# ai4co/rl4co

Measured on NVIDIA H100. Metric: node-selections/sec TSP-100 AM rollout, higher is better.
Workload: dtype f32

## Files before the change

### rl4co_b200/csrc/rollout_impl.cuh

```cuda
#pragma once
#include "co_common.cuh"

namespace co {

#define CO_MODE_GREEDY 0
#define CO_MODE_SAMPLE 1
#define CO_MODE_EVALUATE 2

template <int SPL>
struct Cfg {
  static constexpr int NS = 32 * SPL;
  static constexpr int NW = SPL;
  static constexpr int MINB = SPL == 4 ? 1 : (SPL == 2 ? 2 : 3);
};

constexpr int TILE_LD = 20;

template <int SPL>
struct Smem {
  float ptab[(32 * SPL + 1) * E];
  float qfix[E];
  float wcap[E];
  float hfirst[E];
  float tile[8][32 * TILE_LD];
  alignas(16) float oh[8][D];
  alignas(16) float part[8][32 * SPL];
  alignas(16) float zbuf[2][32 * SPL];
  alignas(16) uint2 red[4];
  alignas(16) float lps[32];
  float dem[32 * SPL];
  float lim[32 * SPL];
  float2 loc[32 * SPL];
  unsigned char order[32 * SPL];
  unsigned char rank_of[32 * SPL];
  alignas(16) float wdyn[3 * E];
  alignas(16) float pwk[32 * SPL * 8 + 8];
};

__device__ __forceinline__ float ex2(float x) {
  float y;
  asm("ex2.approx.ftz.f32 %0, %1;" : "=f"(y) : "f"(x));
  return y;
}
__device__ __forceinline__ float lg2(float x) {
  float y;
  asm("lg2.approx.ftz.f32 %0, %1;" : "=f"(y) : "f"(x));
  return y;
}
__device__ __forceinline__ unsigned fkey(float f) {
  unsigned u = __float_as_uint(f);
  return u ^ ((u >> 31) ? 0xffffffffu : 0x80000000u);
}
__device__ __forceinline__ float funkey(unsigned k) {
  return __uint_as_float(k ^ ((k >> 31) ? 0x80000000u : 0xffffffffu));
}

__device__ __forceinline__ float warp_sum_fixed(float x) {
  constexpr float S = 16777216.f;
  const unsigned hi = __float2uint_rz(x * S);
  const float rem = fmaf(x, S, -(float)hi);
  const unsigned lo = __float2uint_rz(rem * S);
  const unsigned Hs = __reduce_add_sync(FULL, hi), Ls = __reduce_add_sync(FULL, lo);
  return fmaf((float)Ls, 1.0f / (S * S), (float)Hs * (1.0f / S));
}

static __device__ __noinline__ void first_node_gemv(const float* __restrict__ w_first, const float* hfirst, float* qfix, int tid) {
  const int e = tid >> 1, half = tid & 1;
  const float4* wr = reinterpret_cast<const float4*>(w_first + (size_t)e * E + 64 * half);
  const float4* hv = reinterpret_cast<const float4*>(hfirst + 64 * half);
  float s0 = 0.f, s1 = 0.f;
#pragma unroll
  for (int c = 0; c < 16; c += 2) {
    const float4 w0 = __ldg(wr + c), x0 = hv[c], w1 = __ldg(wr + c + 1), x1 = hv[c + 1];
    s0 = fmaf(w0.x, x0.x, s0); s0 = fmaf(w0.y, x0.y, s0); s0 = fmaf(w0.z, x0.z, s0); s0 = fmaf(w0.w, x0.w, s0);
    s1 = fmaf(w1.x, x1.x, s1); s1 = fmaf(w1.y, x1.y, s1); s1 = fmaf(w1.z, x1.z, s1); s1 = fmaf(w1.w, x1.w, s1);
  }
  float sacc = s0 + s1;
  sacc += __shfl_xor_sync(FULL, sacc, 1);
  if (half == 0) qfix[e] += sacc;
}

__device__ __forceinline__ float dist2_fma(float2 a, float2 b) {
  const float dx = a.x - b.x, dy = a.y - b.y;
  return sqrtf(fmaf(dy, dy, dx * dx));
}

template <int ENV>
__device__ __forceinline__ bool feasible(int n, bool visbit, float d, float used, float thr, int cur, bool anyfeas) {
  if (ENV == CO_ENV_TSP) return !visbit;
  if (ENV == CO_ENV_OP) return (n == 0) || (!visbit && !anyfeas && !(d > thr));
  if (ENV == CO_ENV_PCTSP) return (n == 0) ? !((used < 1.0f) && anyfeas) : (!visbit && d == 0.0f);
  if (n == 0) return !(cur == 0 && anyfeas);
  if (ENV == CO_ENV_SDVRP) return !visbit && !(d == 0.0f) && !(used >= thr);
  return !visbit && !((d + used) > thr);
}

template <int SPL, int ENV, int MODE, int CWB>
__global__ void __launch_bounds__(256, Cfg<SPL>::MINB) rollout_kernel(const co_rollout_args A) {
  using C = Cfg<SPL>;
  constexpr int NS = C::NS, NW = C::NW;
  constexpr int CW = CWB * E;
  constexpr int CUR_BLK = CWB - 1;
  constexpr bool first_table = (ENV == CO_ENV_TSP) && (CWB == 5);
  constexpr bool VRP = (ENV != CO_ENV_TSP);
  constexpr bool SD = (ENV == CO_ENV_SDVRP);
  constexpr bool OP = (ENV == CO_ENV_OP);
  constexpr bool PC = (ENV == CO_ENV_PCTSP);
  constexpr float LOG2E = 1.4426950408889634f, LN2 = 0.6931471805599453f;
  extern __shared__ __align__(16) unsigned char smem_raw[];
  Smem<SPL>& sm = *reinterpret_cast<Smem<SPL>*>(smem_raw);

  const int tid = threadIdx.x, lane = tid & 31, h = tid >> 5;
  const int N = A.N, B_inst = A.B_inst, S = A.num_starts, T_max = A.T_max;
  const int B_traj = B_inst * S;
  const bool forced_start = (S > 1) && (A.flags & CO_ROLLOUT_FORCED_START);
  const bool philox = (A.noise == nullptr);
  const bool sel_warp = h < NW;
  const bool lp_warp = h == NW;
  const int nL = sel_warp ? tid : NS - 1;
  const int nG = SPL * lane;
  const float clip = A.tanh_clipping, inv_temp = 1.0f / A.temperature;
  const float Zb = clip * inv_temp;
  float* tile = sm.tile[h];

  float2 Kr[SPL][8], Vr[SPL][8], Lr[SPL][8];

  for (int b = blockIdx.x; b < B_inst; b += gridDim.x) {
    __syncthreads();
    const float* crow = A.cache + (size_t)b * N * CW;
#pragma unroll
    for (int k = 0; k < SPL; ++k) {
      const int n = nG + k;
      if (n < N) {
        const float4* ks = reinterpret_cast<const float4*>(crow + (size_t)n * CW + 0 * E + h * D);
        const float4* vs = reinterpret_cast<const float4*>(crow + (size_t)n * CW + 1 * E + h * D);
        const float4* ls = reinterpret_cast<const float4*>(crow + (size_t)n * CW + 2 * E + h * D);
#pragma unroll
        for (int c = 0; c < 4; ++c) {
          const float4 kv = __ldg(ks + c), vv = __ldg(vs + c), lv = __ldg(ls + c);
          Kr[k][2 * c] = make_float2(kv.x, kv.y); Kr[k][2 * c + 1] = make_float2(kv.z, kv.w);
          Vr[k][2 * c] = make_float2(vv.x, vv.y); Vr[k][2 * c + 1] = make_float2(vv.z, vv.w);
          Lr[k][2 * c] = make_float2(lv.x, lv.y); Lr[k][2 * c + 1] = make_float2(lv.z, lv.w);
        }
      } else {
#pragma unroll
        for (int j = 0; j < 8; ++j) {
          Kr[k][j] = make_float2(0.f, 0.f); Vr[k][j] = make_float2(0.f, 0.f); Lr[k][j] = make_float2(0.f, 0.f);
        }
      }
    }
    for (int idx = tid; idx < N * (E / 4); idx += 256) {
      const int n = idx >> 5, c = idx & 31;
      const uint32_t dst = (uint32_t)__cvta_generic_to_shared(reinterpret_cast<float4*>(sm.ptab + n * E) + c);
      asm volatile("cp.async.cg.shared.global [%0], [%1], 16;" ::"r"(dst),
                   "l"(reinterpret_cast<const float4*>(crow + (size_t)n * CW + CUR_BLK * E) + c) : "memory");
    }
    asm volatile("cp.async.commit_group;" ::: "memory");
    if (tid < E) {
      sm.ptab[NS * E + tid] = 0.f;
      sm.wcap[tid] = VRP ? A.w_capacity[tid] : 0.f;
    }
    if (tid < NS) {
      sm.loc[tid] = (tid < N) ? reinterpret_cast<const float2*>(A.locs)[(size_t)b * N + tid] : make_float2(0.f, 0.f);
      sm.dem[tid] = (VRP && tid >= 1 && tid < N) ? A.demand[(size_t)b * (N - 1) + tid - 1] : 0.f;
      if (OP || PC) sm.lim[tid] = (tid < N) ? A.node_limit[(size_t)b * N + tid] : 0.f;
    }
    if (SD) {
      for (int i = tid; i < 3 * E; i += 256) sm.wdyn[i] = A.dyn_w[i];
    }
    const float cap = (VRP && A.vehicle_capacity) ? A.vehicle_capacity[b] : 1.0f;
    const float thr = SD ? cap : cap + 1e-5f;
    asm volatile("cp.async.wait_group 0;" ::: "memory");
    __syncthreads();
    if (SD) {
      for (int i = tid; i < (NS + 1) * 8; i += 256) {
        const int n = i >> 3, hh = i & 7;
        float acc = 0.f;
        if (n < N) {
#pragma unroll
          for (int c = 0; c < D; ++c) acc = fmaf(sm.ptab[n * E + hh * D + c], sm.wdyn[hh * D + c], acc);
        }
        sm.pwk[i] = acc;
      }
      __syncthreads();
    }
    if (ENV == CO_ENV_CVRP) {
      if (tid >= 1 && tid < N) {
        const float d = sm.dem[tid];
        int rank = 0;
        for (int m = 1; m < N; ++m) {
          const float dm = sm.dem[m];
          rank += (dm < d || (dm == d && m < tid)) ? 1 : 0;
        }
        sm.order[rank] = (unsigned char)tid;
        sm.rank_of[tid] = (unsigned char)rank;
      }
      __syncthreads();
    }
    float dmk0[SPL];
    float2 lck[SPL];
#pragma unroll
    for (int k = 0; k < SPL; ++k) {
      dmk0[k] = OP ? sm.lim[nG + k] : sm.dem[nG + k];
      lck[k] = OP ? sm.loc[nG + k] : make_float2(0.f, 0.f);
    }
    const float dL0 = OP ? sm.lim[nL] : sm.dem[nL];
    const float2 lcL = OP ? sm.loc[nL] : make_float2(0.f, 0.f);
    auto head_dot = [&](const float* vec, float (&out)[SPL]) {
      const float4* vp = reinterpret_cast<const float4*>(vec + h * D);
      float2 a2[SPL];
#pragma unroll
      for (int k = 0; k < SPL; ++k) a2[k] = make_float2(0.f, 0.f);
#pragma unroll
      for (int c = 0; c < 4; ++c) {
        const float4 x = vp[c];
#pragma unroll
        for (int k = 0; k < SPL; ++k) {
          a2[k] = ffma2(make_float2(x.x, x.y), Kr[k][2 * c], a2[k]);
          a2[k] = ffma2(make_float2(x.z, x.w), Kr[k][2 * c + 1], a2[k]);
        }
      }
#pragma unroll
      for (int k = 0; k < SPL; ++k) out[k] = a2[k].x + a2[k].y;
    };
    auto add_first = [&](int a_first) {
      if (first_table) {
        if (tid < E) sm.qfix[tid] += __ldg(crow + (size_t)a_first * CW + 3 * E + tid);
      } else {
        if (tid < E) sm.hfirst[tid] = __ldg(A.node_emb + ((size_t)b * N + a_first) * E + tid);
        __syncthreads();
        first_node_gemv(A.w_first, sm.hfirst, sm.qfix, tid);
      }
    };
    float WK[SPL], FK[SPL];
#pragma unroll
    for (int k = 0; k < SPL; ++k) { WK[k] = 0.f; FK[k] = 0.f; }
    if (VRP) head_dot(sm.wcap, WK);
    float WKW = 0.f, wv_d = 0.f;
    if (SD) {
#pragma unroll
      for (int c = 0; c < D; ++c) WKW = fmaf(sm.wcap[h * D + c], sm.wdyn[h * D + c], WKW);
      wv_d = sm.wdyn[E + h * D + (lane & 15)];
    }
    if (!(A.flags & CO_ROLLOUT_NO_PREFETCH) && b + (int)gridDim.x < B_inst) {
      const char* nxt = reinterpret_cast<const char*>(A.cache + (size_t)(b + gridDim.x) * N * CW);
      for (int i = tid; i < N * 16; i += 256) {
        const int n = i >> 4, blk = (i >> 2) & 3, line = i & 3;
        const size_t off = ((size_t)n * CW + (blk < 3 ? blk : CUR_BLK) * E) * 4 + ((size_t)line << 7);
        asm volatile("prefetch.global.L2 [%0];" ::"l"(nxt + off));
      }
    }

    for (int s = 0; s < S; ++s) {
      const int traj = s * B_inst + b;
      int64_t* act_row = A.actions_out + (size_t)traj * T_max;
      float* lp_row = A.logp_out + (size_t)traj * T_max;
      uint32_t mybits = (!sel_warp || nL >= N) ? 0x100u : 0u;
#pragma unroll
      for (int k = 0; k < SPL; ++k) mybits |= (nG + k >= N) ? (1u << k) : 0u;
      int cur = (ENV == CO_ENV_TSP) ? NS : 0;
      int prev = 0, first = 0, t = 0, dstep = 0, nvis = 0;
      uint32_t rmask[SPL];
#pragma unroll
      for (int k = 0; k < SPL; ++k) {
        const int lo = 32 * k, nc = N - 1;
        rmask[k] = (nc >= lo + 32) ? 0u : (nc <= lo ? 0xffffffffu : (0xffffffffu << (nc - lo)));
      }
      float used = 0.f, dist = 0.f;
      bool anyfeas = false, done = false, depot_seen = false;
      float dmk[SPL], dL = dL0;
#pragma unroll
      for (int k = 0; k < SPL; ++k) dmk[k] = dmk0[k];
      int nrem = 0;
      int pend_a = -1;
      float pend_d = 0.f, FKW = 0.f;
      float ll = 0.f;
      float pen = 0.f;
      if (SD && s > 0 && tid < NS) sm.dem[tid] = (tid >= 1 && tid < N) ? A.demand[(size_t)b * (N - 1) + tid - 1] : 0.f;
      __syncthreads();
      if (tid < E) {
        float g = A.graph_ctx ? A.graph_ctx[(size_t)b * E + tid] : 0.f;
        if (ENV == CO_ENV_TSP && !forced_start) g += A.q_placeholder[tid];
        sm.qfix[tid] = g;
      }

      auto env_step = [&](int a) {
        if (!SD) {
          const unsigned dd = (unsigned)(a - nG);
          mybits |= (dd < (unsigned)SPL) ? (1u << dd) : 0u;
          mybits |= (a == nL) ? 0x100u : 0u;
        }
        if (!OP && h == 0) {
          const float2 pa = sm.loc[a], pp = sm.loc[prev];
          const float dx = pa.x - pp.x, dy = pa.y - pp.y;
          if (VRP || t != 0) dist += sqrtf(dx * dx + dy * dy);
        }
        if (ENV == CO_ENV_TSP) {
          if (t == 0) first = a;
        } else if (OP) {
          used = used + dist2_fma(sm.loc[a], sm.loc[prev]);
          if (h == 0) dist += sm.dem[a];
          depot_seen = depot_seen || (a == 0);
        } else if (PC) {
          used = used + sm.dem[a];
          if (h == 0) pen += sm.lim[a];
          nvis += (a != 0) ? 1 : 0;
          depot_seen = depot_seen || (a == 0);
        } else if (SD) {
          const float d_a = sm.dem[a];
          const float delivered = fminf(d_a, cap - used);
          used = (used + delivered) * (a != 0 ? 1.0f : 0.0f);
          const float d_new = d_a + (-delivered);
#pragma unroll
          for (int k = 0; k < SPL; ++k) dmk[k] = (a == nG + k) ? d_new : dmk[k];
          dL = (a == nL) ? d_new : dL;
          nrem += ((d_new > 0.f) ? 1 : 0) - ((d_a > 0.f) ? 1 : 0);
          pend_a = a; pend_d = d_new;
          anyfeas = (nrem > 0) && !(used >= cap);
        } else {
          used = (used + sm.dem[a == 0 ? 1 : a]) * (a != 0 ? 1.0f : 0.0f);
          nvis += (a != 0 || !depot_seen) ? 1 : 0;
          depot_seen = depot_seen || (a == 0);
          if (a != 0) {
            const int r = sm.rank_of[a];
#pragma unroll
            for (int k = 0; k < SPL; ++k) rmask[k] |= ((r >> 5) == k) ? (1u << (r & 31)) : 0u;
          }
          int pmin = NS;
#pragma unroll
          for (int k = SPL - 1; k >= 0; --k) {
            const uint32_t z = ~rmask[k];
            if (z) pmin = 32 * k + __ffs(z) - 1;
          }
          anyfeas = (pmin < N - 1) && !((sm.dem[sm.order[pmin < N - 1 ? pmin : 0]] + used) > thr);
        }
        prev = a; cur = a; ++t;
        done = (ENV == CO_ENV_TSP) ? (t >= N) : ((OP || PC) ? (a == 0 && t > 1) : (SD ? (nrem == 0) : (nvis >= N)));
      };
      auto logp_of = [&](int buf, int a_sel, int t_out) {
        const float* zb = sm.zbuf[buf];
        float sacc = 0.f;
#pragma unroll
        for (int k = 0; k < SPL; ++k) sacc += ex2((zb[nG + k] - Zb) * LOG2E);
        sm.lps[lane] = sacc;
        __syncwarp();
        const float4* lq = reinterpret_cast<const float4*>(sm.lps);
        const float4 q0 = lq[0], q1 = lq[1], q2 = lq[2], q3 = lq[3], q4 = lq[4], q5 = lq[5], q6 = lq[6], q7 = lq[7];
        const float t0 = ((q0.x + q0.y) + (q0.z + q0.w)) + ((q1.x + q1.y) + (q1.z + q1.w));
        const float t1 = ((q2.x + q2.y) + (q2.z + q2.w)) + ((q3.x + q3.y) + (q3.z + q3.w));
        const float t2 = ((q4.x + q4.y) + (q4.z + q4.w)) + ((q5.x + q5.y) + (q5.z + q5.w));
        const float t3 = ((q6.x + q6.y) + (q6.z + q6.w)) + ((q7.x + q7.y) + (q7.z + q7.w));
        sacc = (t0 + t1) + (t2 + t3);
        __syncwarp();
        const float lp = (zb[a_sel] - Zb) - lg2(sacc) * LN2;
        if (lane == 0) {
          lp_row[t_out] = lp;
          ll += lp;
        }
      };

      if (SD) {
        for (int n = 1; n < N; ++n) nrem += (sm.dem[n] > 0.f) ? 1 : 0;
        anyfeas = (nrem > 0) && !(used >= cap);
        done = (nrem == 0);
      }
      if (forced_start) {
        const int a0 = (s % A.num_loc) + (VRP ? 1 : 0);
        if (tid == 0) { act_row[0] = a0; lp_row[0] = 0.f; }
        env_step(a0);
        if (ENV == CO_ENV_TSP) {
          __syncthreads();
          add_first(a0);
        }
      } else if (ENV == CO_ENV_CVRP) {
        anyfeas = !((sm.dem[sm.order[0]] + used) > thr);
      }
      __syncthreads();
      head_dot(sm.qfix, FK);
      if (SD) {
#pragma unroll
        for (int c = 0; c < D; ++c) FKW = fmaf(sm.qfix[h * D + c], sm.wdyn[h * D + c], FKW);
      }

      while (!done && t < T_max) {
        int forced = 0;
        float gum = 0.f;
        if (MODE == CO_MODE_EVALUATE) forced = (int)A.forced_actions[(size_t)traj * T_max + t];
        if (MODE == CO_MODE_SAMPLE && tid < N) {
          const float q = philox ? philox_exp1(A.seed, A.offset, traj, dstep, tid)
                                 : A.noise[((size_t)dstep * B_traj + traj) * N + tid];
          gum = -logf(q);
        }

        {
          const float4* pr = reinterpret_cast<const float4*>(sm.ptab + cur * E + h * D);
          const float rem = PC ? fmaxf(cap - used, 0.0f) : cap - used;
          float2 sc2[SPL];
#pragma unroll
          for (int k = 0; k < SPL; ++k) sc2[k] = make_float2(0.f, 0.f);
#pragma unroll
          for (int c = 0; c < 4; ++c) {
            const float4 p = pr[c];
#pragma unroll
            for (int k = 0; k < SPL; ++k) {
              sc2[k] = ffma2(make_float2(p.x, p.y), Kr[k][2 * c], sc2[k]);
              sc2[k] = ffma2(make_float2(p.z, p.w), Kr[k][2 * c + 1], sc2[k]);
            }
          }
          float sc[SPL], m = -INFINITY;
          bool fz[SPL];
          const float qwk = SD ? fmaf(rem, WKW, sm.pwk[cur * 8 + h] + FKW) : 0.f;
          const float2 pcur = OP ? sm.loc[cur] : make_float2(0.f, 0.f);
#pragma unroll
          for (int k = 0; k < SPL; ++k) {
            fz[k] = OP ? feasible<ENV>(nG + k, (mybits >> k) & 1u, used + dist2_fma(lck[k], pcur), used, dmk[k], cur, depot_seen)
                    : PC ? feasible<ENV>(nG + k, (mybits >> k) & 1u, depot_seen ? 1.0f : 0.0f, used, thr, cur, nvis < N - 1)
                         : feasible<ENV>(nG + k, (mybits >> k) & 1u, dmk[k], used, thr, cur, anyfeas);
            float dot = (sc2[k].x + sc2[k].y) + FK[k];
            if (VRP) dot = fmaf(rem, WK[k], dot);
            if (SD) dot = fmaf(dmk[k], qwk, dot);
            sc[k] = fz[k] ? dot * (0.25f * LOG2E) : -INFINITY;
            m = fmaxf(m, sc[k]);
          }
          m = funkey(__reduce_max_sync(FULL, fkey(m)));
          float2 acc[8];
          float esum = 0.f, sed = 0.f;
#pragma unroll
          for (int j = 0; j < 8; ++j) acc[j] = make_float2(0.f, 0.f);
#pragma unroll
          for (int k = 0; k < SPL; ++k) {
            const float e = fz[k] ? ex2(sc[k] - m) : 0.f;
            esum += e;
            if (SD) sed = fmaf(e, dmk[k], sed);
            const float2 e2 = make_float2(e, e);
#pragma unroll
            for (int j = 0; j < 8; ++j) acc[j] = ffma2(e2, Vr[k][j], acc[j]);
          }
          float4* trow = reinterpret_cast<float4*>(tile + lane * TILE_LD);
#pragma unroll
          for (int c = 0; c < 4; ++c) trow[c] = make_float4(acc[2 * c].x, acc[2 * c].y, acc[2 * c + 1].x, acc[2 * c + 1].y);
          if (SD) sed = warp_sum(sed);
          __syncwarp();
          const int d = lane & 15, half = lane >> 4;
          float s0 = 0.f, s1 = 0.f, s2 = 0.f, s3 = 0.f;
#pragma unroll
          for (int r = 0; r < 16; r += 4) {
            s0 += tile[(16 * half + ((r + 0 + 4 * half) & 15)) * TILE_LD + d];
            s1 += tile[(16 * half + ((r + 1 + 4 * half) & 15)) * TILE_LD + d];
            s2 += tile[(16 * half + ((r + 2 + 4 * half) & 15)) * TILE_LD + d];
            s3 += tile[(16 * half + ((r + 3 + 4 * half) & 15)) * TILE_LD + d];
          }
          float r = (s0 + s1) + (s2 + s3);
          r += __shfl_xor_sync(FULL, r, 16);
          if (SD) r = fmaf(sed, wv_d, r);
          if (lane < 16) sm.oh[h][lane] = r;
          __syncwarp();
          const float4* op = reinterpret_cast<const float4*>(sm.oh[h]);
          float2 pl2[SPL];
          float olh = 0.f;
#pragma unroll
          for (int k = 0; k < SPL; ++k) pl2[k] = make_float2(0.f, 0.f);
#pragma unroll
          for (int c = 0; c < 4; ++c) {
            const float4 x = op[c];
#pragma unroll
            for (int k = 0; k < SPL; ++k) {
              pl2[k] = ffma2(make_float2(x.x, x.y), Lr[k][2 * c], pl2[k]);
              pl2[k] = ffma2(make_float2(x.z, x.w), Lr[k][2 * c + 1], pl2[k]);
            }
            if (SD) {
              const float4 w = reinterpret_cast<const float4*>(sm.wdyn + 2 * E + h * D)[c];
              olh = fmaf(x.x, w.x, olh); olh = fmaf(x.y, w.y, olh); olh = fmaf(x.z, w.z, olh); olh = fmaf(x.w, w.w, olh);
            }
          }
          esum = warp_sum_fixed(esum);
          const float rinv = __fdividef(1.0f, esum);
          float pl[SPL];
#pragma unroll
          for (int k = 0; k < SPL; ++k) {
            float v = pl2[k].x + pl2[k].y;
            if (SD) v = fmaf(dmk[k], olh, v);
            pl[k] = v * rinv;
          }
          float* pdst = sm.part[h] + nG;
          if (SPL == 4) *reinterpret_cast<float4*>(pdst) = make_float4(pl[0], pl[SPL > 1 ? 1 : 0], pl[SPL > 2 ? 2 : 0], pl[SPL > 3 ? 3 : 0]);
          else if (SPL == 2) *reinterpret_cast<float2*>(pdst) = make_float2(pl[0], pl[SPL > 1 ? 1 : 0]);
          else *pdst = pl[0];
        }
        __syncthreads();

        if (SD && tid == 0 && pend_a >= 0) sm.dem[pend_a] = pend_d;
        if (sel_warp) {
          const bool fzL = OP ? feasible<ENV>(nL, (mybits >> 8) & 1u, used + dist2_fma(lcL, sm.loc[cur]), used, dL, cur, depot_seen)
                           : PC ? feasible<ENV>(nL, (mybits >> 8) & 1u, depot_seen ? 1.0f : 0.0f, used, thr, cur, nvis < N - 1)
                                : feasible<ENV>(nL, (mybits >> 8) & 1u, dL, used, thr, cur, anyfeas);
          const float p = ((sm.part[0][nL] + sm.part[1][nL]) + (sm.part[2][nL] + sm.part[3][nL])) +
                          ((sm.part[4][nL] + sm.part[5][nL]) + (sm.part[6][nL] + sm.part[7][nL]));
          const float lg = tanhf(p * 0.08838834764831845f) * clip;
          const float z = fzL ? lg * inv_temp : -INFINITY;
          sm.zbuf[dstep & 1][nL] = z;
          if (MODE != CO_MODE_EVALUATE) {
            const float keyf = (MODE == CO_MODE_SAMPLE) ? (fzL ? z + gum : -INFINITY) : z;
            const unsigned key = fkey(keyf);
            const unsigned wkey = __reduce_max_sync(FULL, key);
            const unsigned vote = __ballot_sync(FULL, key == wkey);
            if (lane == 0) sm.red[h] = make_uint2(wkey, (unsigned)(32 * h + __ffs(vote) - 1));
          }
        } else if (lp_warp && dstep > 0) {
          logp_of((dstep - 1) & 1, prev, t - 1);
        }
        __syncthreads();
        int a;
        if (MODE == CO_MODE_EVALUATE) {
          a = (forced < 0 || forced >= N) ? 0 : forced;
        } else if (NW == 1) {
          a = (int)sm.red[0].y;
        } else if (NW == 2) {
          const uint4 r0 = reinterpret_cast<const uint4*>(sm.red)[0];
          a = (int)((r0.z > r0.x) ? r0.w : r0.y);
        } else {
          const uint4 r0 = reinterpret_cast<const uint4*>(sm.red)[0], r1 = reinterpret_cast<const uint4*>(sm.red)[1];
          const bool b01 = r0.z > r0.x, b23 = r1.z > r1.x;
          const unsigned ka = b01 ? r0.z : r0.x, ia = b01 ? r0.w : r0.y;
          const unsigned kb = b23 ? r1.z : r1.x, ib = b23 ? r1.w : r1.y;
          a = (int)((kb > ka) ? ib : ia);
        }
        if (tid == 0) act_row[t] = a;

        const bool was_first = (ENV == CO_ENV_TSP) && (t == 0);
        env_step(a);
        ++dstep;
        if (was_first) {
          if (tid < E) sm.qfix[tid] = A.graph_ctx ? A.graph_ctx[(size_t)b * E + tid] : 0.f;
          __syncthreads();
          add_first(a);
          __syncthreads();
          head_dot(sm.qfix, FK);
        }
      }

      __syncthreads();
      if (lp_warp) {
        if (dstep > 0) logp_of((dstep - 1) & 1, prev, t - 1);
        if (lane == 0) A.loglik_out[traj] = ll;
      }
      if (tid == 0) {
        const float2 pa = sm.loc[(ENV == CO_ENV_TSP) ? first : 0], pp = sm.loc[prev];
        const float dx = pa.x - pp.x, dy = pa.y - pp.y;
        float rw = OP ? dist : -(dist + sqrtf(dx * dx + dy * dy));
        if (PC) {
          float total = 0.f;
          for (int n = 1; n < N; ++n) total += sm.lim[n];
          rw = pen - (-rw + total);
        }
        A.reward_out[traj] = rw;
        if (A.steps_out) A.steps_out[traj] = t;
        if (A.used_capacity_out) A.used_capacity_out[traj] = used;
        if (A.max_steps_out) atomicMax(A.max_steps_out, t);
      }
      for (int c = t + tid; c < T_max; c += 256) { act_row[c] = 0; lp_row[c] = 0.f; }
    }
  }
}

template <int SPL, int ENV, int MODE, int CWB>
static int launch(const co_rollout_args& A, cudaStream_t st) {
  auto kern = rollout_kernel<SPL, ENV, MODE, CWB>;
  const size_t smem = sizeof(Smem<SPL>);
  static PerDeviceOnce once;
  static int ctas_per_sm = 1;
  bool& configured = once.flag();
  if (!configured) {
    cudaError_t e = cudaFuncSetAttribute(kern, cudaFuncAttributeMaxDynamicSharedMemorySize, (int)smem);
    if (e != cudaSuccess) return fail(CO_ERR_CUDA, "co_rollout: smem attribute: %s", cudaGetErrorString(e));
    e = cudaOccupancyMaxActiveBlocksPerMultiprocessor(&ctas_per_sm, kern, 256, smem);
    if (e != cudaSuccess || ctas_per_sm < 1) return fail(CO_ERR_CUDA, "co_rollout: occupancy query failed%s");
    configured = true;
  }
  int grid = device_info().sm_count * ctas_per_sm;
  if (grid > A.B_inst) grid = A.B_inst;
  kern<<<grid, 256, smem, st>>>(A);
  return check_launch("co_rollout");
}

template <int ENV>
static int dispatch(const co_rollout_args& A, cudaStream_t st) {
  const int spl = A.N <= 32 ? 1 : (A.N <= 64 ? 2 : 4);
  const int mode = A.select_mode == CO_SELECT_GREEDY ? CO_MODE_GREEDY
                   : (A.select_mode == CO_SELECT_EVALUATE ? CO_MODE_EVALUATE : CO_MODE_SAMPLE);
  const int cwb = A.cache_width / E;
#define CO_CASE(S_, M_)                                                                      \
  if (spl == S_ && mode == M_) {                                                             \
    if (cwb == 4) return launch<S_, ENV, M_, 4>(A, st);                                      \
    if (ENV == CO_ENV_TSP && cwb == 5) return launch<S_, ENV, M_, (ENV == CO_ENV_TSP ? 5 : 4)>(A, st); \
  }
  CO_CASE(1, CO_MODE_GREEDY) CO_CASE(2, CO_MODE_GREEDY) CO_CASE(4, CO_MODE_GREEDY)
  CO_CASE(1, CO_MODE_SAMPLE) CO_CASE(2, CO_MODE_SAMPLE) CO_CASE(4, CO_MODE_SAMPLE)
  CO_CASE(1, CO_MODE_EVALUATE) CO_CASE(2, CO_MODE_EVALUATE) CO_CASE(4, CO_MODE_EVALUATE)
#undef CO_CASE
  return fail(CO_ERR_BAD_ARG, "co_rollout: no kernel variant%s");
}

}
```

### rl4co_b200/csrc/rollout_tsp.cu

```cuda
#include "rollout_impl.cuh"
namespace co {
int rollout_tsp(const co_rollout_args& A, cudaStream_t st) { return dispatch<CO_ENV_TSP>(A, st); }
}
```

### rl4co_b200/native.py

```python

from __future__ import annotations

import ctypes
import os
import subprocess
import sys
from ctypes import POINTER, Structure, c_char_p, c_float, c_int, c_int32, c_uint64, c_void_p

import torch

_HERE = os.path.dirname(os.path.abspath(__file__))
CSRC = os.path.join(_HERE, "csrc")
INCLUDE = os.path.join(os.path.dirname(_HERE), "include")
LIB_PATH = os.path.join(_HERE, "libcorollout.so")
SOURCES = ["abi.cu", "env_kernels.cu", "decode_step.cu", "rollout.cu", "rollout_tsp.cu", "rollout_cvrp.cu", "rollout_ms_tsp.cu", "rollout_ms_cvrp.cu", "rollout_sdvrp.cu", "rollout_op.cu", "rollout_pctsp.cu", "gemm_tf32x3.cu",
           "encoder_mha.cu", "encoder_mha_wgmma.cu",
           "ffn_fused.cu", "data_kernels.cu", "attn_train.cu", "norm_kernels.cu", "op_kernels.cu", "local_search.cu"]
HEADERS = ["co_common.cuh", "rollout_impl.cuh", "rollout_ms_impl.cuh", "wgmma.cuh"]

CO_OK = 0
ENV_TSP, ENV_CVRP = 0, 1
ENV_SDVRP = 2
ENV_OP, ENV_PCTSP = 3, 4
ENV_KIND = {"tsp": ENV_TSP, "cvrp": ENV_CVRP, "sdvrp": ENV_SDVRP, "op": ENV_OP, "pctsp": ENV_PCTSP}
ROLLOUT_ENVS = ("tsp", "cvrp", "sdvrp", "op", "pctsp")
SELECT_GREEDY, SELECT_SAMPLE_NOISE, SELECT_EVALUATE, SELECT_SAMPLE_PHILOX = 0, 1, 2, 3
ROLLOUT_FORCED_START = 1
EMBED_DIM, NUM_HEADS = 128, 8

EXPORTS = [
    "co_version", "co_last_error_string", "co_device_sm_count", "co_tsp_step", "co_cvrp_action_mask",
    "co_cvrp_step", "co_tour_length", "co_check_tours", "co_pointer_logits", "co_select_action",
    "co_cache_width", "co_rollout_max_nodes", "co_rollout", "co_reward_stats", "co_split_tf32", "co_gemm_tf32x3", "co_encoder_mha",
    "co_ffn_fused", "co_ffn_tile_weights", "co_ffn_tiled_weight_floats", "co_generate_uniform", "co_generate_demand", "co_dihedral8",
    "co_sdvrp_step", "co_sdvrp_action_mask", "co_attn_fwd", "co_attn_bwd", "co_instance_norm", "co_op_step", "co_op_action_mask", "co_op_reward", "co_pctsp_step", "co_pctsp_action_mask",
    "co_tsp_two_opt",
]


class NativeLibraryError(RuntimeError):
    pass


class DecoderWeights(Structure):
    _fields_ = [("project_context_t", c_void_p), ("w_placeholder", c_void_p), ("project_out_t", c_void_p),
                ("dynamic_w", c_void_p), ("dynamic_feature", c_void_p)]


class RolloutArgs(Structure):
    _fields_ = [
        ("env_kind", c_int32), ("select_mode", c_int32), ("B_inst", c_int32), ("num_starts", c_int32),
        ("N", c_int32), ("T_max", c_int32), ("num_loc", c_int32), ("flags", c_int32),
        ("tanh_clipping", c_float), ("temperature", c_float),
        ("cache", c_void_p), ("graph_ctx", c_void_p), ("q_placeholder", c_void_p), ("w_capacity", c_void_p),
        ("locs", c_void_p), ("demand", c_void_p), ("vehicle_capacity", c_void_p),
        ("forced_actions", c_void_p), ("noise", c_void_p), ("seed", c_uint64), ("offset", c_uint64),
        ("actions_out", c_void_p), ("logp_out", c_void_p), ("reward_out", c_void_p), ("loglik_out", c_void_p),
        ("steps_out", c_void_p), ("max_steps_out", c_void_p), ("used_capacity_out", c_void_p),
        ("node_emb", c_void_p), ("w_first", c_void_p), ("cache_width", c_int32), ("reserved0", c_int32),
        ("dyn_w", c_void_p), ("node_limit", c_void_p),
    ]


class AttnArgs(Structure):
    _fields_ = ([(n, c_void_p) for n in ("q", "k", "v", "mask", "o", "lse", "dO", "dq", "dk", "dv")]
                + [(n, c_int32) for n in ("B", "M", "N", "reserved0")]
                + [(n, ctypes.c_int64) for n in ("q_bs", "k_bs", "v_bs", "o_bs", "dq_bs", "dk_bs", "dv_bs")]
                + [(n, c_int32) for n in ("q_rs", "k_rs", "v_rs", "o_rs", "dq_rs", "dk_rs", "dv_rs")]
                + [("scale", c_float)])


NVCC_FLAGS = ["-gencode", "arch=compute_90a,code=sm_90a", "-O3", "-lineinfo", "-std=c++17",
              "-Xcompiler", "-fPIC", "-I", INCLUDE]


def _nvcc() -> str:
    nvcc = os.environ.get("NVCC", "/usr/local/cuda/bin/nvcc")
    return nvcc if os.path.exists(nvcc) else "nvcc"


def build(force: bool = False, verbose: bool = False, extra_flags: list[str] | None = None) -> str:
    deps = [os.path.join(CSRC, s) for s in SOURCES + HEADERS] + [os.path.join(INCLUDE, "corollout.h")]
    if not force and os.path.exists(LIB_PATH) and all(os.path.getmtime(LIB_PATH) >= os.path.getmtime(s) for s in deps):
        return LIB_PATH
    objdir = os.path.join(_HERE, "build")
    os.makedirs(objdir, exist_ok=True)
    procs = []
    for s in SOURCES:
        obj = os.path.join(objdir, s.replace(".cu", ".o"))
        cmd = [_nvcc()] + NVCC_FLAGS + (extra_flags or []) + ["-c", os.path.join(CSRC, s), "-o", obj]
        if verbose:
            print(" ".join(cmd), file=sys.stderr)
        procs.append((s, obj, subprocess.Popen(cmd, stdout=subprocess.PIPE, stderr=subprocess.STDOUT, text=True)))
    objs, log = [], []
    for s, obj, p in procs:
        out, _ = p.communicate()
        log.append(out)
        if p.returncode != 0:
            raise NativeLibraryError(f"nvcc failed on {s} ({p.returncode}):\n{out}")
        objs.append(obj)
    link = [_nvcc(), "-gencode", "arch=compute_90a,code=sm_90a", "-shared", "-o", LIB_PATH] + objs
    res = subprocess.run(link, capture_output=True, text=True)
    if res.returncode != 0:
        raise NativeLibraryError(f"link failed ({res.returncode}):\n{res.stdout}\n{res.stderr}")
    build.last_log = "\n".join(log)
    return LIB_PATH


_lib = None


def lib() -> ctypes.CDLL:
    global _lib
    if _lib is not None:
        return _lib
    if not os.path.exists(LIB_PATH):
        raise NativeLibraryError(
            f"{LIB_PATH} not found: run `python -c 'import __graft_entry__ as g; g.build()'` "
            "(there is no CPU/PyTorch fallback for the rollout path)")
    L = ctypes.CDLL(LIB_PATH)
    for name in EXPORTS:
        if not hasattr(L, name):
            raise NativeLibraryError(f"{LIB_PATH} does not export {name}")
    L.co_last_error_string.restype = c_char_p
    L.co_rollout.argtypes = [POINTER(RolloutArgs), c_void_p]
    L.co_pointer_logits.argtypes = [c_int, POINTER(DecoderWeights)] + [c_void_p] * 12 + [c_int, c_int, c_int, c_int, c_void_p]
    L.co_select_action.argtypes = [c_void_p] * 6 + [c_int, c_float, c_float, c_int, c_uint64, c_uint64, c_int, c_int, c_void_p]
    L.co_tsp_step.argtypes = [c_void_p] * 7 + [c_int, c_int, c_void_p]
    L.co_cvrp_action_mask.argtypes = [c_void_p] * 6 + [c_int, c_int, c_void_p]
    L.co_cvrp_step.argtypes = [c_void_p] * 10 + [c_int, c_int, c_void_p]
    L.co_tour_length.argtypes = [c_void_p] * 3 + [c_int] * 5 + [c_void_p]
    L.co_sdvrp_action_mask.argtypes = [c_void_p] * 5 + [c_int, c_int, c_void_p]
    L.co_sdvrp_step.argtypes = [c_void_p] * 9 + [c_int, c_int, c_void_p]
    L.co_check_tours.argtypes = [c_void_p] * 4 + [c_int] * 4 + [c_void_p]
    L.co_tsp_two_opt.argtypes = [c_void_p] * 5 + [c_int] * 3 + [c_void_p]
    L.co_reward_stats.argtypes = [c_void_p, c_void_p, c_int, c_void_p]
    L.co_op_action_mask.argtypes = [c_void_p] * 6 + [c_int, c_int, c_void_p]
    L.co_op_step.argtypes = [c_void_p] * 12 + [c_int, c_int, c_void_p]
    L.co_pctsp_action_mask.argtypes = [c_void_p] * 3 + [c_int, c_int, c_void_p]
    L.co_pctsp_step.argtypes = [c_void_p] * 11 + [c_int, c_int, c_void_p]
    L.co_op_reward.argtypes = [c_void_p] * 3 + [c_int, c_int, c_int, c_void_p]
    L.co_instance_norm.argtypes = [c_void_p, c_void_p, c_void_p, c_void_p, ctypes.c_long, c_int, c_float, c_void_p]
    L.co_attn_fwd.argtypes = [POINTER(AttnArgs), c_void_p]
    L.co_attn_bwd.argtypes = [POINTER(AttnArgs), c_void_p]
    L.co_cache_width.argtypes = [c_int]
    L.co_split_tf32.argtypes = [c_void_p, c_void_p, c_void_p, ctypes.c_long, c_void_p]
    L.co_gemm_tf32x3.argtypes = [c_void_p] * 8 + [c_int] * 7 + [c_void_p]
    L.co_encoder_mha.argtypes = [c_void_p, c_void_p, c_int, c_int, c_void_p]
    L.co_ffn_fused.argtypes = [c_void_p] * 7 + [c_int, c_int, c_int, c_void_p]
    L.co_ffn_tile_weights.argtypes = [c_void_p] * 5 + [c_void_p]
    L.co_ffn_tiled_weight_floats.restype = ctypes.c_long
    L.co_generate_uniform.argtypes = [c_void_p, ctypes.c_long, c_uint64, c_uint64, c_float, c_float, c_void_p]
    L.co_generate_demand.argtypes = [c_void_p, ctypes.c_long, c_uint64, c_uint64, c_int, c_int, c_float, c_void_p]
    L.co_dihedral8.argtypes = [c_void_p, c_void_p, ctypes.c_long, c_int, c_void_p]
    _lib = L
    return L


LAUNCH_COUNT = 0


def _check(rc: int, what: str) -> None:
    global LAUNCH_COUNT
    LAUNCH_COUNT += 1
    if rc != CO_OK:
        msg = lib().co_last_error_string().decode("utf-8", "replace")
        raise NativeLibraryError(f"{what} failed with code {rc}: {msg}")


def _ptr(t: torch.Tensor | None, dtype: torch.dtype | None = None, name: str = "tensor", strided: bool = False):
    if t is None:
        return None
    if not isinstance(t, torch.Tensor):
        raise TypeError(f"{name}: expected a torch.Tensor, got {type(t)}")
    if not t.is_cuda:
        raise NativeLibraryError(f"{name}: libcorollout needs CUDA tensors (got device {t.device}); "
                                 "there is no CPU fallback")
    if dtype is not None and t.dtype != dtype:
        raise TypeError(f"{name}: expected dtype {dtype}, got {t.dtype}")
    if not strided and not t.is_contiguous():
        raise ValueError(f"{name}: tensor must be contiguous")
    return t.data_ptr()


def _stream():
    return torch.cuda.current_stream().cuda_stream


def _on_device_of_first_tensor(fn):
    import functools

    @functools.wraps(fn)
    def wrapper(*args, **kwargs):
        for a in list(args) + list(kwargs.values()):
            if isinstance(a, torch.Tensor) and a.is_cuda:
                if a.device.index != torch.cuda.current_device():
                    with torch.cuda.device(a.device):
                        return fn(*args, **kwargs)
                break
        return fn(*args, **kwargs)

    return wrapper


F32, I64, U8, I32 = torch.float32, torch.int64, torch.uint8, torch.int32


def _bool_ptr(t, name):
    if t is None:
        return None
    if t.dtype not in (torch.bool, torch.uint8):
        raise TypeError(f"{name}: expected bool/uint8, got {t.dtype}")
    return _ptr(t, None, name)




def version() -> int:
    return lib().co_version()


def cache_width(env_name: str) -> int:
    return lib().co_cache_width(ENV_KIND[env_name])


def rollout_max_nodes() -> int:
    return lib().co_rollout_max_nodes()


@_on_device_of_first_tensor
def tsp_step(action, mask_in, mask_out, first_node, current_node, i, done):
    B, N = mask_in.shape
    _check(lib().co_tsp_step(_ptr(action, I64, "action"), _bool_ptr(mask_in, "mask_in"), _bool_ptr(mask_out, "mask_out"),
                             _ptr(first_node, I64, "first_node"), _ptr(current_node, I64, "current_node"),
                             _ptr(i, I64, "i"), _bool_ptr(done, "done"), B, N, _stream()), "co_tsp_step")


@_on_device_of_first_tensor
def cvrp_action_mask(demand, used, cap, visited, current_node, mask_out):
    B, N = visited.shape
    _check(lib().co_cvrp_action_mask(_ptr(demand, F32, "demand"), _ptr(used, F32, "used"), _ptr(cap, F32, "cap"),
                                     _ptr(visited, U8, "visited"), _ptr(current_node, I64, "current_node"),
                                     _bool_ptr(mask_out, "mask_out"), B, N, _stream()), "co_cvrp_action_mask")


@_on_device_of_first_tensor
def cvrp_step(action, demand, cap, used_in, used_out, visited_in, visited_out, current_node, done, mask_out):
    B, N = visited_in.shape
    _check(lib().co_cvrp_step(_ptr(action, I64, "action"), _ptr(demand, F32, "demand"), _ptr(cap, F32, "cap"),
                              _ptr(used_in, F32, "used_in"), _ptr(used_out, F32, "used_out"),
                              _ptr(visited_in, U8, "visited_in"), _ptr(visited_out, U8, "visited_out"),
                              _ptr(current_node, I64, "current_node"), _bool_ptr(done, "done"),
                              _bool_ptr(mask_out, "mask_out"), B, N, _stream()), "co_cvrp_step")


@_on_device_of_first_tensor
def sdvrp_action_mask(demand_with_depot, used, cap, current_node, mask_out):
    B, N = demand_with_depot.shape
    _check(lib().co_sdvrp_action_mask(_ptr(demand_with_depot, F32, "demand_with_depot"), _ptr(used, F32, "used_capacity"),
                                      _ptr(cap, F32, "vehicle_capacity"), _ptr(current_node, I64, "current_node"),
                                      _bool_ptr(mask_out, "mask_out"), B, N, _stream()), "co_sdvrp_action_mask")
    return mask_out


@_on_device_of_first_tensor
def sdvrp_step(action, demand_in, demand_out, cap, used_in, used_out, current_node, done, mask_out):
    B, N = demand_in.shape
    _check(lib().co_sdvrp_step(_ptr(action, I64, "action"), _ptr(demand_in, F32, "demand_in"),
                               _ptr(demand_out, F32, "demand_out"), _ptr(cap, F32, "vehicle_capacity"),
                               _ptr(used_in, F32, "used_in"), _ptr(used_out, F32, "used_out"),
                               _ptr(current_node, I64, "current_node"), _bool_ptr(done, "done"),
                               _bool_ptr(mask_out, "mask_out"), B, N, _stream()), "co_sdvrp_step")


@_on_device_of_first_tensor
def op_action_mask(locs, max_length, visited, tour_length, current_node, mask_out):
    B, N = mask_out.shape
    _check(lib().co_op_action_mask(_ptr(locs, F32, "locs"), _ptr(max_length, F32, "max_length"), _bool_ptr(visited, "visited"),
                                   _ptr(tour_length, F32, "tour_length"), _ptr(current_node, I64, "current_node"),
                                   _bool_ptr(mask_out, "mask_out"), B, N, _stream()), "co_op_action_mask")
    return mask_out


@_on_device_of_first_tensor
def op_step(action, locs, prize, max_length, visited_in, visited_out, tour_length, current_total_prize, current_node, i,
            done, mask_out):
    B, N = mask_out.shape
    _check(lib().co_op_step(_ptr(action, I64, "action"), _ptr(locs, F32, "locs"), _ptr(prize, F32, "prize"),
                            _ptr(max_length, F32, "max_length"), _bool_ptr(visited_in, "visited_in"),
                            _bool_ptr(visited_out, "visited_out"), _ptr(tour_length, F32, "tour_length"),
                            _ptr(current_total_prize, F32, "current_total_prize"), _ptr(current_node, I64, "current_node"),
                            _ptr(i, I64, "i"), _bool_ptr(done, "done"), _bool_ptr(mask_out, "mask_out"), B, N, _stream()),
           "co_op_step")


@_on_device_of_first_tensor
def pctsp_action_mask(visited, cur_total_prize, mask_out):
    B, N = mask_out.shape
    _check(lib().co_pctsp_action_mask(_bool_ptr(visited, "visited"), _ptr(cur_total_prize, F32, "cur_total_prize"),
                                      _bool_ptr(mask_out, "mask_out"), B, N, _stream()), "co_pctsp_action_mask")
    return mask_out


@_on_device_of_first_tensor
def pctsp_step(action, real_prize, penalty, visited_in, visited_out, cur_total_prize, cur_total_penalty, current_node, i, done,
               mask_out):
    B, N = mask_out.shape
    _check(lib().co_pctsp_step(_ptr(action, I64, "action"), _ptr(real_prize, F32, "real_prize"), _ptr(penalty, F32, "penalty"),
                               _bool_ptr(visited_in, "visited_in"), _bool_ptr(visited_out, "visited_out"),
                               _ptr(cur_total_prize, F32, "cur_total_prize"), _ptr(cur_total_penalty, F32, "cur_total_penalty"),
                               _ptr(current_node, I64, "current_node"), _ptr(i, I64, "i"), _bool_ptr(done, "done"),
                               _bool_ptr(mask_out, "mask_out"), B, N, _stream()), "co_pctsp_step")


@_on_device_of_first_tensor
def op_reward(prize, actions):
    B, T = actions.shape
    if prize.shape[0] != B:
        prize = prize.repeat(B // prize.shape[0], 1)
    out = torch.empty(B, dtype=F32, device=actions.device)
    _check(lib().co_op_reward(_ptr(prize.contiguous(), F32, "prize"), _ptr(actions, I64, "actions"), _ptr(out, F32, "reward"),
                              B, prize.shape[1], T, _stream()), "co_op_reward")
    return out


@_on_device_of_first_tensor
def tour_length(locs, actions, with_depot: bool):
    B, T = actions.shape
    B_locs, N = locs.shape[0], locs.shape[1]
    reward = torch.empty(B, dtype=F32, device=actions.device)
    _check(lib().co_tour_length(_ptr(locs, F32, "locs"), _ptr(actions, I64, "actions"), _ptr(reward, F32, "reward"),
                                B, B_locs, N, T, int(with_depot), _stream()), "co_tour_length")
    return reward


@_on_device_of_first_tensor
def check_tours(actions, N, demand=None, cap=None, B_inst=None) -> int:
    B, T = actions.shape
    bad = torch.zeros(1, dtype=I32, device=actions.device)
    _check(lib().co_check_tours(_ptr(actions, I64, "actions"), _ptr(demand, F32, "demand"), _ptr(cap, F32, "cap"),
                                _ptr(bad, I32, "bad"), B, B if B_inst is None else B_inst, N, T, _stream()),
           "co_check_tours")
    return int(bad.item())


@_on_device_of_first_tensor
def tsp_two_opt(tours, max_iterations: int = 1000, locs=None, distances=None, iterations=None):
    if (locs is None) == (distances is None):
        raise ValueError("tsp_two_opt: pass exactly one of locs / distances")
    if tours.dim() != 2:
        raise ValueError(f"tours: expected [B, N], got {tuple(tours.shape)}")
    B, N = tours.shape
    if locs is not None and tuple(locs.shape) != (B, N, 2):
        raise ValueError(f"locs: expected [{B}, {N}, 2], got {tuple(locs.shape)}")
    if distances is not None and tuple(distances.shape) != (B, N, N):
        raise ValueError(f"distances: expected [{B}, {N}, {N}], got {tuple(distances.shape)}")
    if iterations is not None and tuple(iterations.shape) != (B,):
        raise ValueError(f"iterations: expected [{B}], got {tuple(iterations.shape)}")
    out = torch.empty(B, N, dtype=I64, device=tours.device)
    _check(lib().co_tsp_two_opt(_ptr(locs, F32, "locs"), _ptr(distances, F32, "distances"), _ptr(tours, I64, "tours"),
                                _ptr(out, I64, "tours_out"), _ptr(iterations, I32, "iterations"), B, N,
                                min(int(max_iterations), 2**31 - 1), _stream()), "co_tsp_two_opt")
    return out


@_on_device_of_first_tensor
def pointer_logits(env_name, weights: DecoderWeights, node_emb, graph_ctx, K, V, L, mask, first_node, current_node,
                   i, used, cap, B_traj, B_inst, N):
    ld = K.stride(1)
    for name, x in (("glimpse_key", K), ("glimpse_val", V), ("logit_key", L)):
        if x.stride(2) != 1 or x.stride(1) != ld or x.stride(0) != N * ld:
            raise ValueError(f"{name}: unsupported strides {x.stride()}")
    logits = torch.empty(B_traj, N, dtype=F32, device=node_emb.device)
    _check(lib().co_pointer_logits(ENV_KIND["cvrp" if env_name in ("op", "pctsp") else env_name], ctypes.byref(weights), _ptr(node_emb, F32, "node_emb"),
                                   _ptr(graph_ctx, F32, "graph_ctx"), _ptr(K, F32, "glimpse_key", True),
                                   _ptr(V, F32, "glimpse_val", True), _ptr(L, F32, "logit_key", True),
                                   _bool_ptr(mask, "action_mask"), _ptr(first_node, I64, "first_node"),
                                   _ptr(current_node, I64, "current_node"), _ptr(i, I64, "i"),
                                   _ptr(used, F32, "used_capacity"), _ptr(cap, F32, "vehicle_capacity"),
                                   _ptr(logits, F32, "logits"), B_traj, B_inst, N, ld, _stream()), "co_pointer_logits")
    return logits


@_on_device_of_first_tensor
def select_action(logits, mask, mode, noise=None, action=None, tanh_clipping=10.0, temperature=1.0,
                  mask_logits=True, store_all_logp=False, seed=0, offset=0):
    B, N = logits.shape
    if action is None:
        action = torch.empty(B, dtype=I64, device=logits.device)
    logp = torch.empty(B, dtype=F32, device=logits.device)
    all_lp = torch.empty(B, N, dtype=F32, device=logits.device) if store_all_logp else None
    _check(lib().co_select_action(_ptr(logits, F32, "logits"), _bool_ptr(mask, "mask"), _ptr(noise, F32, "noise"),
                                  _ptr(action, I64, "action"), _ptr(logp, F32, "logp"), _ptr(all_lp, F32, "logprobs"),
                                  mode, float(tanh_clipping), float(temperature), int(mask_logits), seed, offset,
                                  B, N, _stream()), "co_select_action")
    return action, logp, all_lp


@_on_device_of_first_tensor
def split_tf32(w: torch.Tensor):
    w = w.detach().contiguous()
    hi, lo = torch.empty_like(w), torch.empty_like(w)
    _check(lib().co_split_tf32(_ptr(w, F32, "w"), _ptr(hi, F32, "hi"), _ptr(lo, F32, "lo"), w.numel(), _stream()),
           "co_split_tf32")
    return hi, lo


@_on_device_of_first_tensor
def gemm_tf32x3(a, w_hi, w_lo, out=None, bias=None, residual=None, scale=None, shift=None, relu=False):
# ... 198 lines not shown
```

Measured before the change: 103.7 million.

## Split log-prob and reward work across idle warps in a pipelined schedule

```diff
diff --git a/rl4co_b200/csrc/rollout_impl.cuh b/rl4co_b200/csrc/rollout_impl.cuh
--- a/rl4co_b200/csrc/rollout_impl.cuh
+++ b/rl4co_b200/csrc/rollout_impl.cuh
@@ -27,7 +27,7 @@
   alignas(16) float part[8][32 * SPL];
   alignas(16) float zbuf[2][32 * SPL];
   alignas(16) uint2 red[4];
-  alignas(16) float lps[32];
+  alignas(16) float lps[2][36];
   float dem[32 * SPL];
   float lim[32 * SPL];
   float2 loc[32 * SPL];
@@ -36,6 +36,29 @@
   alignas(16) float wdyn[3 * E];
   alignas(16) float pwk[32 * SPL * 8 + 8];
 };
+
+enum { CO_PH_SCORES, CO_PH_SOFTMAX_AV, CO_PH_TRANSPOSE, CO_PH_POINTER, CO_PH_B1, CO_PH_SELECT, CO_PH_B2, CO_PH_MERGE_ENV,
+       CO_PROF_PHASES };
+#ifdef CO_ROLLOUT_PHASE_PROF
+constexpr int CO_PROF_CTAS = 4;
+static __device__ unsigned long long co_phase_cycles[CO_PROF_CTAS][2][CO_PROF_PHASES + 1];
+#define CO_PROF_DECL                                                                      \
+  const bool prof_on = blockIdx.x < CO_PROF_CTAS && (h == 0 || h == 4);                   \
+  unsigned prof_t = 0;
+#define CO_PROF_START() \
+  if (prof_on) prof_t = (unsigned)clock();
+#define CO_PROF_MARK(p)                                                                          \
+  if (prof_on) {                                                                                 \
+    const unsigned prof_now = (unsigned)clock();                                                 \
+    if (lane == 0) atomicAdd(&co_phase_cycles[blockIdx.x][h >> 2][p], (unsigned long long)(prof_now - prof_t)); \
+    if (lane == 0 && (p) == CO_PH_MERGE_ENV) atomicAdd(&co_phase_cycles[blockIdx.x][h >> 2][CO_PROF_PHASES], 1ull); \
+    prof_t = prof_now;                                                                           \
+  }
+#else
+#define CO_PROF_DECL
+#define CO_PROF_START()
+#define CO_PROF_MARK(p)
+#endif
 
 __device__ __forceinline__ float ex2(float x) {
   float y;
@@ -117,11 +140,14 @@
   const bool philox = (A.noise == nullptr);
   const bool sel_warp = h < NW;
   const bool lp_warp = h == NW;
+  const bool tl_warp = h == NW + 1;
+  const bool ll_warp = h == NW + 2;
   const int nL = sel_warp ? tid : NS - 1;
   const int nG = SPL * lane;
   const float clip = A.tanh_clipping, inv_temp = 1.0f / A.temperature;
   const float Zb = clip * inv_temp;
   float* tile = sm.tile[h];
+  CO_PROF_DECL
 
   float2 Kr[SPL][8], Vr[SPL][8], Lr[SPL][8];
 
@@ -260,13 +286,15 @@
       for (int k = 0; k < SPL; ++k) mybits |= (nG + k >= N) ? (1u << k) : 0u;
       int cur = (ENV == CO_ENV_TSP) ? NS : 0;
       int prev = 0, first = 0, t = 0, dstep = 0, nvis = 0;
+      int tl_prev = 0;
       uint32_t rmask[SPL];
 #pragma unroll
       for (int k = 0; k < SPL; ++k) {
         const int lo = 32 * k, nc = N - 1;
         rmask[k] = (nc >= lo + 32) ? 0u : (nc <= lo ? 0xffffffffu : (0xffffffffu << (nc - lo)));
       }
-      float used = 0.f, dist = 0.f;
+      float used = 0.f;
+      float dist = 0.f;
       bool anyfeas = false, done = false, depot_seen = false;
       float dmk[SPL], dL = dL0;
 #pragma unroll
@@ -290,20 +318,13 @@
           mybits |= (dd < (unsigned)SPL) ? (1u << dd) : 0u;
           mybits |= (a == nL) ? 0x100u : 0u;
         }
-        if (!OP && h == 0) {
-          const float2 pa = sm.loc[a], pp = sm.loc[prev];
-          const float dx = pa.x - pp.x, dy = pa.y - pp.y;
-          if (VRP || t != 0) dist += sqrtf(dx * dx + dy * dy);
-        }
         if (ENV == CO_ENV_TSP) {
           if (t == 0) first = a;
         } else if (OP) {
           used = used + dist2_fma(sm.loc[a], sm.loc[prev]);
-          if (h == 0) dist += sm.dem[a];
           depot_seen = depot_seen || (a == 0);
         } else if (PC) {
           used = used + sm.dem[a];
-          if (h == 0) pen += sm.lim[a];
           nvis += (a != 0) ? 1 : 0;
           depot_seen = depot_seen || (a == 0);
         } else if (SD) {
@@ -337,22 +358,32 @@
         prev = a; cur = a; ++t;
         done = (ENV == CO_ENV_TSP) ? (t >= N) : ((OP || PC) ? (a == 0 && t > 1) : (SD ? (nrem == 0) : (nvis >= N)));
       };
-      auto logp_of = [&](int buf, int a_sel, int t_out) {
+      auto reward_step = [&](int a, int p, int ta) {
+        if (!OP) {
+          const float2 pa = sm.loc[a], pp = sm.loc[p];
+          const float dx = pa.x - pp.x, dy = pa.y - pp.y;
+          if (VRP || ta != 0) dist += sqrtf(dx * dx + dy * dy);
+        }
+        if (OP) dist += sm.dem[a];
+        if (PC) pen += sm.lim[a];
+      };
+      auto lp_expsum = [&](int buf, int a_sel) {
         const float* zb = sm.zbuf[buf];
         float sacc = 0.f;
 #pragma unroll
         for (int k = 0; k < SPL; ++k) sacc += ex2((zb[nG + k] - Zb) * LOG2E);
-        sm.lps[lane] = sacc;
-        __syncwarp();
-        const float4* lq = reinterpret_cast<const float4*>(sm.lps);
+        sm.lps[buf][lane] = sacc;
+        if (lane == 0) sm.lps[buf][32] = zb[a_sel];
+      };
+      auto lp_finish = [&](int buf, int t_out) {
+        const float4* lq = reinterpret_cast<const float4*>(sm.lps[buf]);
         const float4 q0 = lq[0], q1 = lq[1], q2 = lq[2], q3 = lq[3], q4 = lq[4], q5 = lq[5], q6 = lq[6], q7 = lq[7];
         const float t0 = ((q0.x + q0.y) + (q0.z + q0.w)) + ((q1.x + q1.y) + (q1.z + q1.w));
         const float t1 = ((q2.x + q2.y) + (q2.z + q2.w)) + ((q3.x + q3.y) + (q3.z + q3.w));
         const float t2 = ((q4.x + q4.y) + (q4.z + q4.w)) + ((q5.x + q5.y) + (q5.z + q5.w));
         const float t3 = ((q6.x + q6.y) + (q6.z + q6.w)) + ((q7.x + q7.y) + (q7.z + q7.w));
-        sacc = (t0 + t1) + (t2 + t3);
-        __syncwarp();
-        const float lp = (zb[a_sel] - Zb) - lg2(sacc) * LN2;
+        const float sacc = (t0 + t1) + (t2 + t3);
+        const float lp = (sm.lps[buf][32] - Zb) - lg2(sacc) * LN2;
         if (lane == 0) {
           lp_row[t_out] = lp;
           ll += lp;
@@ -382,6 +413,7 @@
         for (int c = 0; c < D; ++c) FKW = fmaf(sm.qfix[h * D + c], sm.wdyn[h * D + c], FKW);
       }
 
+      CO_PROF_START()
       while (!done && t < T_max) {
         int forced = 0;
         float gum = 0.f;
@@ -423,6 +455,7 @@
             m = fmaxf(m, sc[k]);
           }
           m = funkey(__reduce_max_sync(FULL, fkey(m)));
+          CO_PROF_MARK(CO_PH_SCORES)
           float2 acc[8];
           float esum = 0.f, sed = 0.f;
 #pragma unroll
@@ -439,6 +472,7 @@
           float4* trow = reinterpret_cast<float4*>(tile + lane * TILE_LD);
 #pragma unroll
           for (int c = 0; c < 4; ++c) trow[c] = make_float4(acc[2 * c].x, acc[2 * c].y, acc[2 * c + 1].x, acc[2 * c + 1].y);
+          CO_PROF_MARK(CO_PH_SOFTMAX_AV)
           if (SD) sed = warp_sum(sed);
           __syncwarp();
           const int d = lane & 15, half = lane >> 4;
@@ -455,6 +489,7 @@
           if (SD) r = fmaf(sed, wv_d, r);
           if (lane < 16) sm.oh[h][lane] = r;
           __syncwarp();
+          CO_PROF_MARK(CO_PH_TRANSPOSE)
           const float4* op = reinterpret_cast<const float4*>(sm.oh[h]);
           float2 pl2[SPL];
           float olh = 0.f;
@@ -486,8 +521,10 @@
           if (SPL == 4) *reinterpret_cast<float4*>(pdst) = make_float4(pl[0], pl[SPL > 1 ? 1 : 0], pl[SPL > 2 ? 2 : 0], pl[SPL > 3 ? 3 : 0]);
           else if (SPL == 2) *reinterpret_cast<float2*>(pdst) = make_float2(pl[0], pl[SPL > 1 ? 1 : 0]);
           else *pdst = pl[0];
+          CO_PROF_MARK(CO_PH_POINTER)
         }
         __syncthreads();
+        CO_PROF_MARK(CO_PH_B1)
 
         if (SD && tid == 0 && pend_a >= 0) sm.dem[pend_a] = pend_d;
         if (sel_warp) {
@@ -507,9 +544,16 @@
             if (lane == 0) sm.red[h] = make_uint2(wkey, (unsigned)(32 * h + __ffs(vote) - 1));
           }
         } else if (lp_warp && dstep > 0) {
-          logp_of((dstep - 1) & 1, prev, t - 1);
-        }
+          lp_expsum((dstep - 1) & 1, prev);
+        } else if (ll_warp && dstep > 1) {
+          lp_finish((dstep - 2) & 1, t - 2);
+        } else if (tl_warp && t > 0) {
+          reward_step(cur, tl_prev, t - 1);
+          tl_prev = cur;
+        }
+        CO_PROF_MARK(CO_PH_SELECT)
         __syncthreads();
+        CO_PROF_MARK(CO_PH_B2)
         int a;
         if (MODE == CO_MODE_EVALUATE) {
           a = (forced < 0 || forced >= N) ? 0 : forced;
@@ -537,14 +581,14 @@
           __syncthreads();
           head_dot(sm.qfix, FK);
         }
+        CO_PROF_MARK(CO_PH_MERGE_ENV)
       }
 
       __syncthreads();
-      if (lp_warp) {
-        if (dstep > 0) logp_of((dstep - 1) & 1, prev, t - 1);
-        if (lane == 0) A.loglik_out[traj] = ll;
-      }
-      if (tid == 0) {
+      if (lp_warp && dstep > 0) lp_expsum((dstep - 1) & 1, prev);
+      if (ll_warp && dstep > 1) lp_finish((dstep - 2) & 1, t - 2);
+      if (tl_warp && lane == 0) {
+        if (t > 0) reward_step(cur, tl_prev, t - 1);
         const float2 pa = sm.loc[(ENV == CO_ENV_TSP) ? first : 0], pp = sm.loc[prev];
         const float dx = pa.x - pp.x, dy = pa.y - pp.y;
         float rw = OP ? dist : -(dist + sqrtf(dx * dx + dy * dy));
@@ -557,6 +601,11 @@
         if (A.steps_out) A.steps_out[traj] = t;
         if (A.used_capacity_out) A.used_capacity_out[traj] = used;
         if (A.max_steps_out) atomicMax(A.max_steps_out, t);
+      }
+      __syncthreads();
+      if (ll_warp) {
+        if (dstep > 0) lp_finish((dstep - 1) & 1, t - 1);
+        if (lane == 0) A.loglik_out[traj] = ll;
       }
       for (int c = t + tid; c < T_max; c += 256) { act_row[c] = 0; lp_row[c] = 0.f; }
     }
diff --git a/rl4co_b200/csrc/rollout_tsp.cu b/rl4co_b200/csrc/rollout_tsp.cu
--- a/rl4co_b200/csrc/rollout_tsp.cu
+++ b/rl4co_b200/csrc/rollout_tsp.cu
@@ -2,3 +2,16 @@
 namespace co {
 int rollout_tsp(const co_rollout_args& A, cudaStream_t st) { return dispatch<CO_ENV_TSP>(A, st); }
 }
+
+#ifdef CO_ROLLOUT_PHASE_PROF
+extern "C" int co_rollout_phase_cycles(unsigned long long* host, int count, int reset) {
+  using namespace co;
+  if (count != (int)(sizeof(co_phase_cycles) / sizeof(unsigned long long))) return -1;
+  if (cudaMemcpyFromSymbol(host, co_phase_cycles, sizeof(co_phase_cycles)) != cudaSuccess) return -2;
+  if (reset) {
+    static const unsigned long long zeros[sizeof(co_phase_cycles) / sizeof(unsigned long long)] = {};
+    if (cudaMemcpyToSymbol(co_phase_cycles, zeros, sizeof(zeros)) != cudaSuccess) return -3;
+  }
+  return 0;
+}
+#endif
diff --git a/rl4co_b200/native.py b/rl4co_b200/native.py
--- a/rl4co_b200/native.py
+++ b/rl4co_b200/native.py
@@ -79,11 +79,13 @@
     return nvcc if os.path.exists(nvcc) else "nvcc"
 
 
-def build(force: bool = False, verbose: bool = False, extra_flags: list[str] | None = None) -> str:
+def build(force: bool = False, verbose: bool = False, extra_flags: list[str] | None = None,
+          out_dir: str | None = None) -> str:
+    lib_path = os.path.join(out_dir, "libcorollout.so") if out_dir else LIB_PATH
     deps = [os.path.join(CSRC, s) for s in SOURCES + HEADERS] + [os.path.join(INCLUDE, "corollout.h")]
-    if not force and os.path.exists(LIB_PATH) and all(os.path.getmtime(LIB_PATH) >= os.path.getmtime(s) for s in deps):
-        return LIB_PATH
-    objdir = os.path.join(_HERE, "build")
+    if not force and os.path.exists(lib_path) and all(os.path.getmtime(lib_path) >= os.path.getmtime(s) for s in deps):
+        return lib_path
+    objdir = os.path.join(out_dir or _HERE, "build")
     os.makedirs(objdir, exist_ok=True)
     procs = []
     for s in SOURCES:
@@ -99,12 +101,12 @@
         if p.returncode != 0:
             raise NativeLibraryError(f"nvcc failed on {s} ({p.returncode}):\n{out}")
         objs.append(obj)
-    link = [_nvcc(), "-gencode", "arch=compute_90a,code=sm_90a", "-shared", "-o", LIB_PATH] + objs
+    link = [_nvcc(), "-gencode", "arch=compute_90a,code=sm_90a", "-shared", "-o", lib_path] + objs
     res = subprocess.run(link, capture_output=True, text=True)
     if res.returncode != 0:
         raise NativeLibraryError(f"link failed ({res.returncode}):\n{res.stdout}\n{res.stderr}")
     build.last_log = "\n".join(log)
-    return LIB_PATH
+    return lib_path
 
 
 _lib = None
```

Measured after the change: 109.5 million, median of 6. 5.6% higher.
